# chengzhag/PanFusion

Hardware: NVIDIA B200
Metric: denoise-steps/sec (512x1024 pano + 8x512^2 views, 50-step DDIM) (higher is better)
Workload: dtype bf16

## Files before the change

panfusion_b200/csrc/fmha_tcgen05.cu:

```cuda
#include <stdlib.h>

#include "pf_common.cuh"

namespace pf {

constexpr int FA_BLOCK_M = 128;
constexpr int FA_BLOCK_N = 64;
constexpr int FA_THREADS = 192;
#ifndef PF_FA_POLY_EXP
#define PF_FA_POLY_EXP 0
#endif
#ifndef PF_FA_ALU_PACK
#define PF_FA_ALU_PACK 0
#endif
#ifndef PF_FA_POLY_DEFAULT
#define PF_FA_POLY_DEFAULT 0
#endif
constexpr bool FA_POLY_EXP = PF_FA_POLY_EXP != 0;
constexpr bool FA_ALU_PACK = PF_FA_ALU_PACK != 0;

struct FmhaParams {
  int B, H, Lq, Lk;
  float scale_log2;
  void* out;
  int out_ld;
  const float* bias;
  long long bias_bstride;
  int bias_ld;
  const uint8_t* bias_flags;
  long long flags_bstride;
  int flags_ld;
  const int* tile_off;
};

__device__ __forceinline__ float fast_exp2(float x) {
  float y;
  asm("ex2.approx.ftz.f32 %0, %1;" : "=f"(y) : "f"(x));
  return y;
}

__device__ __forceinline__ float poly_exp2(float x) {
  x = fmaxf(x, -125.0f);
  const float t = x + 12582912.0f;
  const float f = x - (t - 12582912.0f);
  float p = fmaf(f, 0.05517164f, 0.24261112f);
  p = fmaf(p, f, 0.69326099f);
  p = fmaf(p, f, 0.99992807f);
  return __int_as_float(__float_as_int(p) + (__float_as_int(t) << 23));
}

__device__ __forceinline__ void poly_exp2_pair(float x0, float x1, float& y0, float& y1) {
  const f32x2 x = pack_f2(fmaxf(x0, -125.0f), fmaxf(x1, -125.0f));
  const f32x2 magic = pack_f2(12582912.0f, 12582912.0f);
  const f32x2 t = add_f2(x, magic);
  const f32x2 r = add_f2(t, pack_f2(-12582912.0f, -12582912.0f));
  const f32x2 f = fma_f2(r, pack_f2(-1.0f, -1.0f), x);
  f32x2 p = fma_f2(f, pack_f2(0.05517164f, 0.05517164f), pack_f2(0.24261112f, 0.24261112f));
  p = fma_f2(p, f, pack_f2(0.69326099f, 0.69326099f));
  p = fma_f2(p, f, pack_f2(0.99992807f, 0.99992807f));
  float p0, p1, t0, t1;
  unpack_f2(p, p0, p1);
  unpack_f2(t, t0, t1);
  y0 = __int_as_float(__float_as_int(p0) + (__float_as_int(t0) << 23));
  y1 = __int_as_float(__float_as_int(p1) + (__float_as_int(t1) << 23));
}

__device__ __forceinline__ uint32_t pack_bf16_alu(float a, float b) {
  const uint32_t ua = __float_as_uint(a) + 0x8000u, ub = __float_as_uint(b) + 0x8000u;
  return __byte_perm(ua, ub, 0x7632);
}

template <bool BF16>
__device__ __forceinline__ uint32_t pack_prob(float a, float b) {
  if constexpr (BF16) return pack_bf16_alu(a, b);
  else return pack2<false>(a, b);
}

template <int D>
__host__ __device__ constexpr int fa_stages() { return D == 64 ? 2 : 4; }
template <int D>
__host__ __device__ constexpr int fmha_smem_bytes() {
  return FA_BLOCK_M * D * 2 + fa_stages<D>() * 2 * FA_BLOCK_N * D * 2 + FA_BLOCK_M * FA_BLOCK_N * 2 + 256;
}

template <int D, bool BF16, bool HAS_BIAS, int POLY_PAIRS>
__global__ void __launch_bounds__(FA_THREADS, 3)
fmha_fwd_kernel(const __grid_constant__ CUtensorMap tmQ, const __grid_constant__ CUtensorMap tmK,
                const __grid_constant__ CUtensorMap tmV, const FmhaParams p) {
  static_assert(D == 32 || D == 64, "head dim 32 (EPPA) or 64 (SD-2 UNet)");
  constexpr int STAGES = fa_stages<D>();
  constexpr int Q_BYTES = FA_BLOCK_M * D * 2;
  constexpr int KV_BYTES = FA_BLOCK_N * D * 2;
  constexpr int P_BYTES = FA_BLOCK_M * FA_BLOCK_N * 2;
  constexpr uint32_t SW_LAYOUT = (D == 64) ? 2u : 4u;
  constexpr uint32_t SW_ATOM_BYTES = (D == 64) ? 1024u : 512u;
  constexpr int TMEM_COLS = 128;
  constexpr uint32_t TM_S = 0, TM_O = 64;
  constexpr float RESCALE_THRESHOLD = 8.0f;

  extern __shared__ __align__(1024) uint8_t smem[];
  if ((smem_u32(smem) & 1023u) != 0) __trap();
  uint8_t* sQ = smem;
  uint8_t* sKV = sQ + Q_BYTES;
  uint8_t* sP = sKV + STAGES * 2 * KV_BYTES;
  uint64_t* bars = reinterpret_cast<uint64_t*>(sP + P_BYTES);
  uint64_t* q_full = bars;
  uint64_t* kv_full = bars + 1;
  uint64_t* kv_empty = kv_full + STAGES;
  uint64_t* s_full = kv_empty + STAGES;
  uint64_t* s_free = s_full + 1;
  uint64_t* p_full = s_free + 1;
  uint64_t* o_done = p_full + 1;
  uint32_t* tmem_ptr_smem = reinterpret_cast<uint32_t*>(o_done + 1);

  pdl_launch_dependents();
  const int warp = threadIdx.x >> 5, lane = threadIdx.x & 31;
  const int h = blockIdx.x % p.H;
  const int qt = blockIdx.x / p.H;
  const int b = blockIdx.y;
  const int q0 = qt * FA_BLOCK_M;
  const int n_tiles = (p.Lk + FA_BLOCK_N - 1) / FA_BLOCK_N;

  if (warp == 0 && lane == 0) {
    tma_prefetch_desc(&tmQ);
    tma_prefetch_desc(&tmK);
    tma_prefetch_desc(&tmV);
    mbar_init(q_full, 1);
    for (int s = 0; s < STAGES; ++s) {
      mbar_init(&kv_full[s], 1);
      mbar_init(&kv_empty[s], 1);
    }
    mbar_init(s_full, 1);
    mbar_init(s_free, 128);
    mbar_init(p_full, 128);
    mbar_init(o_done, 1);
    fence_barrier_init();
  }
  if (warp == 1) {
    tmem_alloc(tmem_ptr_smem, TMEM_COLS);
    tmem_relinquish();
  }
  tc_fence_before();
  __syncthreads();
  tc_fence_after();
  const uint32_t tmem_base = *tmem_ptr_smem;
  pdl_wait();

  if (warp == 0) {
    if (lane == 0) {
      mbar_expect_tx(q_full, Q_BYTES);
      tma_load_4d(sQ, &tmQ, q_full, 0, h, q0, b);
      for (int j = 0; j < n_tiles; ++j) {
        const int s = j % STAGES;
        mbar_wait(&kv_empty[s], ((j / STAGES) & 1) ^ 1);
        mbar_expect_tx(&kv_full[s], 2 * KV_BYTES);
        uint8_t* dst = sKV + s * 2 * KV_BYTES;
        tma_load_4d(dst, &tmK, &kv_full[s], 0, h, j * FA_BLOCK_N, b);
        tma_load_4d(dst + KV_BYTES, &tmV, &kv_full[s], 0, h, j * FA_BLOCK_N, b);
      }
    }
  } else if (warp == 1) {
    if (lane == 0) {
      constexpr uint32_t idesc_qk = make_idesc_f16(BF16 ? 1 : 0, FA_BLOCK_M, FA_BLOCK_N, 0, 0);
      constexpr uint32_t idesc_pv = make_idesc_f16(BF16 ? 1 : 0, FA_BLOCK_M, D, 0, 1);
      const uint64_t qdesc = make_smem_desc(smem_u32(sQ), 16, SW_ATOM_BYTES, SW_LAYOUT);
      const uint64_t pdesc = make_smem_desc(smem_u32(sP), 16, 1024, 2);
      auto issue_qk = [&](int j) {
        const int s = j % STAGES;
        mbar_wait(&kv_full[s], (j / STAGES) & 1);
        tc_fence_after();
        const uint64_t kdesc = make_smem_desc(smem_u32(sKV + s * 2 * KV_BYTES), 16, SW_ATOM_BYTES, SW_LAYOUT);
#pragma unroll
        for (int k = 0; k < D / 16; ++k) umma_f16(tmem_base + TM_S, qdesc + 2 * k, kdesc + 2 * k, idesc_qk, k != 0);
        umma_commit(s_full);
      };
      mbar_wait(q_full, 0);
      issue_qk(0);
      for (int j = 0; j < n_tiles; ++j) {
        mbar_wait(s_free, j & 1);
        tc_fence_after();
        if (j + 1 < n_tiles) issue_qk(j + 1);
        mbar_wait(p_full, j & 1);
        tc_fence_after();
        const int s = j % STAGES;
        const uint64_t vdesc =
            make_smem_desc(smem_u32(sKV + s * 2 * KV_BYTES + KV_BYTES), SW_ATOM_BYTES, SW_ATOM_BYTES, SW_LAYOUT);
#pragma unroll
        for (int k = 0; k < FA_BLOCK_N / 16; ++k) {
          umma_f16(tmem_base + TM_O, pdesc + 2 * k, vdesc + uint64_t((2 * SW_ATOM_BYTES * k) >> 4), idesc_pv,
                   (j | k) != 0 ? 1u : 0u);
        }
        umma_commit(o_done);
        umma_commit(&kv_empty[s]);
      }
    }
  } else {
    const int quarter = warp & 3;
    const int row = quarter * 32 + lane;
    const int q = q0 + row;
    const uint32_t lane_addr = tmem_base + (uint32_t(quarter * 32) << 16);
    constexpr float LOG2E = 1.4426950408889634f;
    float m_used = -INFINITY, l_run = 0.f;
    const float* bias_row = nullptr;
    const uint8_t* flag_row = nullptr;
    const int* off_row = nullptr;
    if constexpr (HAS_BIAS) {
      const int qq = q < p.Lq ? q : p.Lq - 1;
      if (p.tile_off) {
        off_row = p.tile_off + (long long)b * p.flags_bstride + (long long)qt * p.flags_ld;
        bias_row = p.bias + (quarter * (FA_BLOCK_N / 4) * 32 + lane) * 4;
      } else {
        bias_row = p.bias + (long long)b * p.bias_bstride + (long long)qq * p.bias_ld;
        if (p.bias_flags) flag_row = p.bias_flags + (long long)b * p.flags_bstride + (long long)qt * p.flags_ld;
      }
    }

    for (int j = 0; j < n_tiles; ++j) {
      const int k0 = j * FA_BLOCK_N;
      int toff = 0;
      if constexpr (HAS_BIAS) {
        if (off_row) toff = off_row[j];
      }
      mbar_wait(s_full, j & 1);
      tc_fence_after();
      float sv[FA_BLOCK_N];
      {
        uint32_t raw[32];
        tmem_ld32(lane_addr + TM_S, raw);
        tmem_ld_wait();
#pragma unroll
        for (int e = 0; e < 32; ++e) sv[e] = __uint_as_float(raw[e]);
        tmem_ld32(lane_addr + TM_S + 32, raw);
        tmem_ld_wait();
#pragma unroll
        for (int e = 0; e < 32; ++e) sv[32 + e] = __uint_as_float(raw[e]);
      }
      tc_fence_before();
      mbar_arrive(s_free);
      float sc = p.scale_log2, shift = 0.f;
      if constexpr (HAS_BIAS) {
        const bool constant_tile = off_row ? toff < 0 : (flag_row != nullptr && flag_row[j] != 0);
        if (constant_tile) {
          shift = -LOG2E;
        } else if (off_row || k0 + FA_BLOCK_N <= p.Lk) {
          const float4* b4 = off_row ? reinterpret_cast<const float4*>(bias_row + (long long)toff * (FA_BLOCK_M * FA_BLOCK_N))
                                     : reinterpret_cast<const float4*>(bias_row + k0);
          const int st4 = off_row ? 32 : 1;
#pragma unroll
          for (int e = 0; e < FA_BLOCK_N / 4; ++e) {
            const float4 t = __ldg(b4 + e * st4);
            sv[4 * e + 0] = fmaf(t.x, LOG2E, sv[4 * e + 0] * p.scale_log2);
            sv[4 * e + 1] = fmaf(t.y, LOG2E, sv[4 * e + 1] * p.scale_log2);
            sv[4 * e + 2] = fmaf(t.z, LOG2E, sv[4 * e + 2] * p.scale_log2);
            sv[4 * e + 3] = fmaf(t.w, LOG2E, sv[4 * e + 3] * p.scale_log2);
          }
          sc = 1.0f;
        } else {
#pragma unroll
          for (int e = 0; e < FA_BLOCK_N; ++e) {
            const float bv = (k0 + e < p.Lk) ? __ldg(bias_row + k0 + e) : 0.f;
            sv[e] = fmaf(bv, LOG2E, sv[e] * p.scale_log2);
          }
          sc = 1.0f;
        }
      }
      if (k0 + FA_BLOCK_N > p.Lk) {
#pragma unroll
        for (int e = 0; e < FA_BLOCK_N; ++e)
          if (k0 + e >= p.Lk) sv[e] = -INFINITY;
      }
      float mxs[8];
#pragma unroll
      for (int i = 0; i < 8; ++i) mxs[i] = sv[i];
#pragma unroll
      for (int e = 8; e < FA_BLOCK_N; ++e) mxs[e & 7] = fmaxf(mxs[e & 7], sv[e]);
      const float mx_raw = fmaxf(fmaxf(fmaxf(mxs[0], mxs[1]), fmaxf(mxs[2], mxs[3])),
                                 fmaxf(fmaxf(mxs[4], mxs[5]), fmaxf(mxs[6], mxs[7])));
      const float mx_tile = HAS_BIAS ? fmaf(mx_raw, sc, shift) : sc * mx_raw;
      const bool need = mx_tile > m_used + RESCALE_THRESHOLD;
      bool o_waited = false;
      if (__any_sync(0xffffffffu, need)) {
        const float m_new = need ? mx_tile : m_used;
        const float alpha = fast_exp2(m_used - m_new);
        if (j > 0) {
          mbar_wait(o_done, (j - 1) & 1);
          tc_fence_after();
          o_waited = true;
          uint32_t raw[16];
#pragma unroll 1
          for (int c = 0; c < D; c += 16) {
            tmem_ld16(lane_addr + TM_O + c, raw);
            tmem_ld_wait();
#pragma unroll
            for (int e = 0; e < 16; ++e) raw[e] = __float_as_uint(__uint_as_float(raw[e]) * alpha);
            tmem_st16(lane_addr + TM_O + c, raw);
          }
          tmem_st_wait();
        }
        l_run *= alpha;
        m_used = m_new;
      }
      f32x2 ps2[4];
#pragma unroll
      for (int i = 0; i < 4; ++i) ps2[i] = pack_f2(0.f, 0.f);
      const f32x2 sc2 = pack_f2(sc, sc), nm2 = HAS_BIAS ? pack_f2(shift - m_used, shift - m_used) : pack_f2(-m_used, -m_used);
      uint32_t pk[FA_BLOCK_N / 2];
#pragma unroll
      for (int e = 0; e < FA_BLOCK_N; e += 2) {
        float a0, a1;
        unpack_f2(fma_f2(pack_f2(sv[e], sv[e + 1]), sc2, nm2), a0, a1);
        float p0, p1;
        if (((e >> 1) & 7) < POLY_PAIRS) {
          poly_exp2_pair(a0, a1, p0, p1);
        } else {
          p0 = fast_exp2(a0);
          p1 = (FA_POLY_EXP && ((e >> 1) & 1)) ? poly_exp2(a1) : fast_exp2(a1);
        }
        ps2[(e >> 1) & 3] = add_f2(ps2[(e >> 1) & 3], pack_f2(p0, p1));
        pk[e >> 1] = FA_ALU_PACK ? pack_prob<BF16>(p0, p1) : pack2<BF16>(p0, p1);
      }
      {
        float lo, hi;
        unpack_f2(add_f2(add_f2(ps2[0], ps2[1]), add_f2(ps2[2], ps2[3])), lo, hi);
        l_run += lo + hi;
      }
      if (j > 0 && !o_waited) {
        mbar_wait(o_done, (j - 1) & 1);
        tc_fence_after();
      }
      {
        uint8_t* prow = sP + row * 128;
#pragma unroll
        for (int c = 0; c < 8; ++c) {
          uint4 v = make_uint4(pk[4 * c], pk[4 * c + 1], pk[4 * c + 2], pk[4 * c + 3]);
          *reinterpret_cast<uint4*>(prow + ((c ^ (row & 7)) << 4)) = v;
        }
      }
      fence_proxy_async_smem();
      tc_fence_before();
      mbar_arrive(p_full);
    }
    mbar_wait(o_done, (n_tiles - 1) & 1);
    tc_fence_after();
    {
      const float inv = 1.0f / l_run;
      uint16_t* orow = static_cast<uint16_t*>(p.out) + ((long long)b * p.Lq + q) * p.out_ld + h * D;
      uint32_t raw[32];
#pragma unroll
      for (int c = 0; c < D; c += 32) {
        tmem_ld32(lane_addr + TM_O + c, raw);
        tmem_ld_wait();
        if (q < p.Lq) {
#pragma unroll
          for (int e = 0; e < 32; e += 8) {
            uint4 v = make_uint4(pack2<BF16>(__uint_as_float(raw[e]) * inv, __uint_as_float(raw[e + 1]) * inv),
                                 pack2<BF16>(__uint_as_float(raw[e + 2]) * inv, __uint_as_float(raw[e + 3]) * inv),
                                 pack2<BF16>(__uint_as_float(raw[e + 4]) * inv, __uint_as_float(raw[e + 5]) * inv),
                                 pack2<BF16>(__uint_as_float(raw[e + 6]) * inv, __uint_as_float(raw[e + 7]) * inv));
            *reinterpret_cast<uint4*>(orow + c + e) = v;
          }
        }
      }
    }
    tc_fence_before();
  }
  __syncthreads();
  if (warp == 1) {
    tc_fence_after();
    tmem_dealloc(tmem_base, TMEM_COLS);
  }
}

static int make_qkv_tmap(CUtensorMap* tm, int dtype, const void* ptr, int B, int H, int L, int D, int ld,
                         long long bstride, int box_rows) {
  uint64_t dims[4] = {(uint64_t)D, (uint64_t)H, (uint64_t)L, (uint64_t)B};
  uint64_t str[3] = {(uint64_t)D * 2, (uint64_t)ld * 2, (uint64_t)bstride * 2};
  uint32_t box[4] = {(uint32_t)D, 1, (uint32_t)box_rows, 1};
  return make_tmap(tm, dtype, 4, ptr, dims, str, box, D == 64 ? 128 : 64);
}

template <int D, bool BF16, bool HAS_BIAS, int POLY_PAIRS>
static int launch_fmha(const pf_fmha_args* a, cudaStream_t st) {
  CUtensorMap tmQ, tmK, tmV;
  int rc;
  if ((rc = make_qkv_tmap(&tmQ, a->dtype, a->q, a->B, a->H, a->Lq, D, a->q_ld, a->q_bstride, FA_BLOCK_M))) return rc;
  if ((rc = make_qkv_tmap(&tmK, a->dtype, a->k, a->B, a->H, a->Lk, D, a->k_ld, a->k_bstride, FA_BLOCK_N))) return rc;
  if ((rc = make_qkv_tmap(&tmV, a->dtype, a->v, a->B, a->H, a->Lk, D, a->v_ld, a->v_bstride, FA_BLOCK_N))) return rc;
  FmhaParams p;
  p.B = a->B; p.H = a->H; p.Lq = a->Lq; p.Lk = a->Lk;
  p.scale_log2 = a->scale * 1.4426950408889634f;
  p.out = a->out; p.out_ld = a->out_ld;
  p.bias = a->bias; p.bias_bstride = a->bias_bstride; p.bias_ld = a->bias_ld;
  p.bias_flags = a->bias_flags; p.flags_bstride = a->flags_bstride; p.flags_ld = a->flags_ld;
  p.tile_off = a->bias_tile_off;
  auto kern = fmha_fwd_kernel<D, BF16, HAS_BIAS, POLY_PAIRS>;
  constexpr int SMEM = fmha_smem_bytes<D>();
  static bool attr_set = false;
  if (!attr_set) {
    rc = check_cuda(cudaFuncSetAttribute(kern, cudaFuncAttributeMaxDynamicSharedMemorySize, SMEM),
                    "cudaFuncSetAttribute(fmha)");
    if (rc) return rc;
    attr_set = true;
  }
  dim3 grid(((a->Lq + FA_BLOCK_M - 1) / FA_BLOCK_M) * a->H, a->B);
  if ((rc = check_cuda(launch_pdl(kern, grid, dim3(FA_THREADS), SMEM, st, tmQ, tmK, tmV, p), "launch(fmha)"))) return rc;
  PF_CHECK_LAUNCH("fmha_fwd_kernel");
  return PF_OK;
}

}

extern "C" int pf_fmha_fwd(const pf_fmha_args* a, void* stream) {
  using namespace pf;
  PF_CHECK_ARG(a != nullptr, "pf_fmha_fwd: null args");
  PF_CHECK_ARG(a->dtype == PF_BF16 || a->dtype == PF_F16, "pf_fmha_fwd: dtype must be PF_F16 or PF_BF16");
  PF_CHECK_ARG(a->q && a->k && a->v && a->out, "pf_fmha_fwd: null operand");
  PF_CHECK_ARG(a->head_dim == 32 || a->head_dim == 64, "pf_fmha_fwd: head_dim %d unsupported (32 or 64)", a->head_dim);
  PF_CHECK_ARG(a->B > 0 && a->B <= 65535 && a->H > 0 && a->Lq > 0 && a->Lk > 0, "pf_fmha_fwd: empty shape");
  PF_CHECK_ARG(a->q_ld % 8 == 0 && a->k_ld % 8 == 0 && a->v_ld % 8 == 0 && a->out_ld % 8 == 0,
               "pf_fmha_fwd: leading dims must be multiples of 8 elements");
  PF_CHECK_ARG(((uintptr_t)a->q & 15) == 0 && ((uintptr_t)a->k & 15) == 0 && ((uintptr_t)a->v & 15) == 0 &&
                   ((uintptr_t)a->out & 15) == 0,
               "pf_fmha_fwd: operands must be 16-byte aligned");
  PF_CHECK_ARG(!a->bias || a->bias_tile_off || (a->bias_ld % 4 == 0 && ((uintptr_t)a->bias & 15) == 0 && a->bias_ld >= a->Lk),
               "pf_fmha_fwd: bias must be 16-byte aligned with bias_ld %% 4 == 0");
  PF_CHECK_ARG(!a->bias_tile_off || (a->bias && ((uintptr_t)a->bias & 15) == 0 && !a->bias_flags && a->flags_ld > 0),
               "pf_fmha_fwd: a tile-packed bias needs the packed store in `bias`, flags_ld = tiles per row, no bias_flags");
  cudaStream_t st = static_cast<cudaStream_t>(stream);
  const bool bf = a->dtype == PF_BF16;
  const bool hb = a->bias != nullptr;
  static const int poly = [] {
    const char* e = getenv("PF_FA_POLY");
    return e ? atoi(e) : PF_FA_POLY_DEFAULT;
  }();
  if (a->head_dim == 64) {
    if (bf && !hb) {
      switch (poly) {
        case 2: return launch_fmha<64, true, false, 2>(a, st);
        case 3: return launch_fmha<64, true, false, 3>(a, st);
        case 4: return launch_fmha<64, true, false, 4>(a, st);
        default: return launch_fmha<64, true, false, 0>(a, st);
      }
    }
    if (bf) return launch_fmha<64, true, true, 0>(a, st);
    return hb ? launch_fmha<64, false, true, 0>(a, st) : launch_fmha<64, false, false, 0>(a, st);
  }
  if (bf) {
    if (hb) {
      switch (poly) {
        case 2: return launch_fmha<32, true, true, 2>(a, st);
        case 3: return launch_fmha<32, true, true, 3>(a, st);
        default: return launch_fmha<32, true, true, 0>(a, st);
      }
    }
    return launch_fmha<32, true, false, 0>(a, st);
  }
  return hb ? launch_fmha<32, false, true, 0>(a, st) : launch_fmha<32, false, false, 0>(a, st);
}
```

panfusion_b200/csrc/pf_common.cuh:

```cuda
#pragma once
#include <cuda.h>
#include <cuda_runtime.h>
#include <cuda_bf16.h>
#include <cuda_fp16.h>
#include <stdint.h>
#include <stdio.h>

#include "../../include/panfusion_b200.h"

namespace pf {

void set_error(const char* fmt, ...);
int  check_cuda(cudaError_t e, const char* what);
bool pdl_enabled();

#define PF_CHECK_ARG(cond, ...)                      \
  do {                                               \
    if (!(cond)) {                                   \
      ::pf::set_error(__VA_ARGS__);                  \
      return PF_ERR_INVALID;                         \
    }                                                \
  } while (0)

#define PF_CHECK_LAUNCH(what)                                         \
  do {                                                                \
    int _rc = ::pf::check_cuda(cudaGetLastError(), what);             \
    if (_rc) return _rc;                                              \
  } while (0)

int make_tmap(CUtensorMap* out, int dtype , int rank, const void* base,
              const uint64_t* dims, const uint64_t* strides_bytes, const uint32_t* box,
              int swizzle_bytes );

#ifdef __CUDACC__

__device__ __forceinline__ uint32_t smem_u32(const void* p) {
  return static_cast<uint32_t>(__cvta_generic_to_shared(p));
}

__device__ __forceinline__ void mbar_init(uint64_t* bar, uint32_t count) {
  asm volatile("mbarrier.init.shared::cta.b64 [%0], %1;" ::"r"(smem_u32(bar)), "r"(count) : "memory");
}
__device__ __forceinline__ void fence_barrier_init() {
  asm volatile("fence.mbarrier_init.release.cluster;" ::: "memory");
}
__device__ __forceinline__ void fence_proxy_async_smem() {
  asm volatile("fence.proxy.async.shared::cta;" ::: "memory");
}
__device__ __forceinline__ void mbar_expect_tx(uint64_t* bar, uint32_t bytes) {
  asm volatile("mbarrier.arrive.expect_tx.shared::cta.b64 _, [%0], %1;" ::"r"(smem_u32(bar)), "r"(bytes)
               : "memory");
}
__device__ __forceinline__ void mbar_arrive(uint64_t* bar) {
  asm volatile("mbarrier.arrive.shared::cta.b64 _, [%0];" ::"r"(smem_u32(bar)) : "memory");
}
__device__ __forceinline__ bool mbar_try_wait(uint64_t* bar, uint32_t parity) {
  uint32_t ok;
  asm volatile(
      "{\n\t.reg .pred p;\n\t"
      "mbarrier.try_wait.parity.shared::cta.b64 p, [%1], %2;\n\t"
      "selp.u32 %0, 1, 0, p;\n\t}"
      : "=r"(ok)
      : "r"(smem_u32(bar)), "r"(parity)
      : "memory");
  return ok != 0;
}
__device__ __forceinline__ void mbar_wait(uint64_t* bar, uint32_t parity) {
  if (mbar_try_wait(bar, parity)) return;
  const long long t0 = clock64();
  while (!mbar_try_wait(bar, parity)) {
    if (clock64() - t0 > 4000000000LL) {
      printf("pf: mbarrier wait timeout (block %d,%d thread %d)\n", blockIdx.x, blockIdx.y, threadIdx.x);
      __trap();
    }
  }
}

__device__ __forceinline__ void tma_prefetch_desc(const CUtensorMap* t) {
  asm volatile("prefetch.tensormap [%0];" ::"l"(t) : "memory");
}
__device__ __forceinline__ void tma_load_2d(void* dst, const CUtensorMap* t, uint64_t* bar, int c0, int c1) {
  asm volatile(
      "cp.async.bulk.tensor.2d.shared::cluster.global.mbarrier::complete_tx::bytes [%0], [%1, {%3, %4}], [%2];"
      ::"r"(smem_u32(dst)), "l"(t), "r"(smem_u32(bar)), "r"(c0), "r"(c1)
      : "memory");
}
__device__ __forceinline__ void tma_load_4d(void* dst, const CUtensorMap* t, uint64_t* bar, int c0, int c1,
                                            int c2, int c3) {
  asm volatile(
      "cp.async.bulk.tensor.4d.shared::cluster.global.mbarrier::complete_tx::bytes [%0], [%1, {%3, %4, %5, %6}], "
      "[%2];" ::"r"(smem_u32(dst)),
      "l"(t), "r"(smem_u32(bar)), "r"(c0), "r"(c1), "r"(c2), "r"(c3)
      : "memory");
}
__device__ __forceinline__ void tma_store_2d(const CUtensorMap* t, const void* src, int c0, int c1) {
  asm volatile("cp.async.bulk.tensor.2d.global.shared::cta.bulk_group [%0, {%2, %3}], [%1];" ::"l"(t),
               "r"(smem_u32(src)), "r"(c0), "r"(c1)
               : "memory");
}
__device__ __forceinline__ void tma_store_commit() { asm volatile("cp.async.bulk.commit_group;" ::: "memory"); }
__device__ __forceinline__ void tma_store_wait_read() { asm volatile("cp.async.bulk.wait_group.read 0;" ::: "memory"); }
__device__ __forceinline__ void named_bar_sync(int id, int nthreads) {
  asm volatile("bar.sync %0, %1;" ::"r"(id), "r"(nthreads) : "memory");
}

__device__ __forceinline__ void bulk_load_1d(void* dst, const void* src, uint32_t bytes, uint64_t* bar) {
  asm volatile(
      "cp.async.bulk.shared::cluster.global.mbarrier::complete_tx::bytes [%0], [%1], %2, [%3];" ::"r"(
          smem_u32(dst)),
      "l"(src), "r"(bytes), "r"(smem_u32(bar))
      : "memory");
}

__device__ __forceinline__ void tmem_alloc(uint32_t* smem_dst, uint32_t ncols) {
  asm volatile("tcgen05.alloc.cta_group::1.sync.aligned.shared::cta.b32 [%0], %1;" ::"r"(smem_u32(smem_dst)),
               "r"(ncols)
               : "memory");
}
__device__ __forceinline__ void tmem_relinquish() {
  asm volatile("tcgen05.relinquish_alloc_permit.cta_group::1.sync.aligned;" ::: "memory");
}
__device__ __forceinline__ void tmem_dealloc(uint32_t taddr, uint32_t ncols) {
  asm volatile("tcgen05.dealloc.cta_group::1.sync.aligned.b32 %0, %1;" ::"r"(taddr), "r"(ncols) : "memory");
}
__device__ __forceinline__ void tc_fence_before() {
  asm volatile("tcgen05.fence::before_thread_sync;" ::: "memory");
}
__device__ __forceinline__ void tc_fence_after() {
  asm volatile("tcgen05.fence::after_thread_sync;" ::: "memory");
}
__device__ __forceinline__ void umma_f16(uint32_t tmem_d, uint64_t adesc, uint64_t bdesc, uint32_t idesc,
                                         uint32_t accumulate) {
  asm volatile(
      "{\n\t.reg .pred p;\n\t"
      "setp.ne.b32 p, %4, 0;\n\t"
      "tcgen05.mma.cta_group::1.kind::f16 [%0], %1, %2, %3, p;\n\t}"
      ::"r"(tmem_d), "l"(adesc), "l"(bdesc), "r"(idesc), "r"(accumulate)
      : "memory");
}
__device__ __forceinline__ void umma_commit(uint64_t* bar) {
  asm volatile("tcgen05.commit.cta_group::1.mbarrier::arrive::one.shared::cluster.b64 [%0];" ::"r"(smem_u32(bar))
               : "memory");
}
__device__ __forceinline__ void tmem_ld_wait() { asm volatile("tcgen05.wait::ld.sync.aligned;" ::: "memory"); }

__device__ __forceinline__ void tmem_ld16(uint32_t taddr, uint32_t (&v)[16]) {
  asm volatile(
      "tcgen05.ld.sync.aligned.32x32b.x16.b32 {%0, %1, %2, %3, %4, %5, %6, %7, %8, %9, %10, %11, %12, %13, %14, "
      "%15}, [%16];"
      : "=r"(v[0]), "=r"(v[1]), "=r"(v[2]), "=r"(v[3]), "=r"(v[4]), "=r"(v[5]), "=r"(v[6]), "=r"(v[7]),
        "=r"(v[8]), "=r"(v[9]), "=r"(v[10]), "=r"(v[11]), "=r"(v[12]), "=r"(v[13]), "=r"(v[14]), "=r"(v[15])
      : "r"(taddr)
      : "memory");
}
__device__ __forceinline__ void tmem_ld32(uint32_t taddr, uint32_t (&v)[32]) {
  asm volatile(
      "tcgen05.ld.sync.aligned.32x32b.x32.b32 {%0, %1, %2, %3, %4, %5, %6, %7, %8, %9, %10, %11, %12, %13, %14, "
      "%15, %16, %17, %18, %19, %20, %21, %22, %23, %24, %25, %26, %27, %28, %29, %30, %31}, [%32];"
      : "=r"(v[0]), "=r"(v[1]), "=r"(v[2]), "=r"(v[3]), "=r"(v[4]), "=r"(v[5]), "=r"(v[6]), "=r"(v[7]),
        "=r"(v[8]), "=r"(v[9]), "=r"(v[10]), "=r"(v[11]), "=r"(v[12]), "=r"(v[13]), "=r"(v[14]), "=r"(v[15]),
        "=r"(v[16]), "=r"(v[17]), "=r"(v[18]), "=r"(v[19]), "=r"(v[20]), "=r"(v[21]), "=r"(v[22]), "=r"(v[23]),
        "=r"(v[24]), "=r"(v[25]), "=r"(v[26]), "=r"(v[27]), "=r"(v[28]), "=r"(v[29]), "=r"(v[30]), "=r"(v[31])
      : "r"(taddr)
      : "memory");
}

__device__ __forceinline__ void tmem_st32(uint32_t taddr, const uint32_t (&v)[32]) {
  asm volatile(
      "tcgen05.st.sync.aligned.32x32b.x32.b32 [%0], {%1, %2, %3, %4, %5, %6, %7, %8, %9, %10, %11, %12, %13, %14, %15, "
      "%16, %17, %18, %19, %20, %21, %22, %23, %24, %25, %26, %27, %28, %29, %30, %31, %32};"
      ::"r"(taddr), "r"(v[0]), "r"(v[1]), "r"(v[2]), "r"(v[3]), "r"(v[4]), "r"(v[5]), "r"(v[6]), "r"(v[7]), "r"(v[8]),
        "r"(v[9]), "r"(v[10]), "r"(v[11]), "r"(v[12]), "r"(v[13]), "r"(v[14]), "r"(v[15]), "r"(v[16]), "r"(v[17]),
        "r"(v[18]), "r"(v[19]), "r"(v[20]), "r"(v[21]), "r"(v[22]), "r"(v[23]), "r"(v[24]), "r"(v[25]), "r"(v[26]),
        "r"(v[27]), "r"(v[28]), "r"(v[29]), "r"(v[30]), "r"(v[31])
      : "memory");
}
__device__ __forceinline__ void tmem_st16(uint32_t taddr, const uint32_t (&v)[16]) {
  asm volatile(
      "tcgen05.st.sync.aligned.32x32b.x16.b32 [%0], {%1, %2, %3, %4, %5, %6, %7, %8, %9, %10, %11, %12, %13, %14, %15, "
      "%16};" ::"r"(taddr),
      "r"(v[0]), "r"(v[1]), "r"(v[2]), "r"(v[3]), "r"(v[4]), "r"(v[5]), "r"(v[6]), "r"(v[7]), "r"(v[8]), "r"(v[9]),
      "r"(v[10]), "r"(v[11]), "r"(v[12]), "r"(v[13]), "r"(v[14]), "r"(v[15])
      : "memory");
}
__device__ __forceinline__ void tmem_st_wait() { asm volatile("tcgen05.wait::st.sync.aligned;" ::: "memory"); }

__device__ __forceinline__ uint32_t cluster_ctarank() {
  uint32_t r;
  asm volatile("mov.u32 %0, %%cluster_ctarank;" : "=r"(r));
  return r;
}
__device__ __forceinline__ void cluster_sync_all() {
  asm volatile("barrier.cluster.arrive.release.aligned;\n\tbarrier.cluster.wait.acquire.aligned;" ::: "memory");
}
__device__ __forceinline__ void tma_load_2d_2sm(void* dst, const CUtensorMap* t, uint64_t* bar, int c0, int c1) {
  asm volatile(
      "cp.async.bulk.tensor.2d.cta_group::2.shared::cluster.global.mbarrier::complete_tx::bytes [%0], [%1, {%3, %4}], "
      "[%2];" ::"r"(smem_u32(dst)),
      "l"(t), "r"(smem_u32(bar) & 0xFEFFFFFFu), "r"(c0), "r"(c1)
      : "memory");
}
__device__ __forceinline__ void tmem_alloc_2sm(uint32_t* smem_dst, uint32_t ncols) {
  asm volatile("tcgen05.alloc.cta_group::2.sync.aligned.shared::cta.b32 [%0], %1;" ::"r"(smem_u32(smem_dst)),
               "r"(ncols)
               : "memory");
}
__device__ __forceinline__ void tmem_relinquish_2sm() {
  asm volatile("tcgen05.relinquish_alloc_permit.cta_group::2.sync.aligned;" ::: "memory");
}
__device__ __forceinline__ void tmem_dealloc_2sm(uint32_t taddr, uint32_t ncols) {
  asm volatile("tcgen05.dealloc.cta_group::2.sync.aligned.b32 %0, %1;" ::"r"(taddr), "r"(ncols) : "memory");
}
__device__ __forceinline__ void umma_f16_2sm(uint32_t tmem_d, uint64_t adesc, uint64_t bdesc, uint32_t idesc,
                                             uint32_t accumulate) {
  asm volatile(
      "{\n\t.reg .pred p;\n\t"
      "setp.ne.b32 p, %4, 0;\n\t"
      "tcgen05.mma.cta_group::2.kind::f16 [%0], %1, %2, %3, p;\n\t}"
      ::"r"(tmem_d), "l"(adesc), "l"(bdesc), "r"(idesc), "r"(accumulate)
      : "memory");
}
__device__ __forceinline__ void umma_commit_2sm(uint64_t* bar) {
  asm volatile(
      "tcgen05.commit.cta_group::2.mbarrier::arrive::one.shared::cluster.multicast::cluster.b64 [%0], %1;" ::"r"(
          smem_u32(bar)),
      "h"((uint16_t)3)
      : "memory");
}

__host__ __device__ constexpr uint32_t make_idesc_f16(int fmt, int M, int N, int a_mn_major, int b_mn_major) {
  return (1u << 4) | (uint32_t(fmt) << 7) | (uint32_t(fmt) << 10) | (uint32_t(a_mn_major) << 15) |
         (uint32_t(b_mn_major) << 16) | (uint32_t(N >> 3) << 17) | (uint32_t(M >> 4) << 24);
}

__device__ __forceinline__ uint64_t make_smem_desc(uint32_t saddr, uint32_t lbo_bytes, uint32_t sbo_bytes,
                                                   uint32_t layout_type) {
  return uint64_t((saddr & 0x3FFFFu) >> 4) | (uint64_t(lbo_bytes >> 4) << 16) | (uint64_t(sbo_bytes >> 4) << 32) |
         (uint64_t(1) << 46) | (uint64_t(layout_type) << 61);
}

template <typename T>
struct Cvt;
template <>
struct Cvt<float> {
  static __device__ __forceinline__ float to_f(float v) { return v; }
  static __device__ __forceinline__ float from_f(float v) { return v; }
};
template <>
struct Cvt<__nv_bfloat16> {
  static __device__ __forceinline__ float to_f(__nv_bfloat16 v) { return __bfloat162float(v); }
  static __device__ __forceinline__ __nv_bfloat16 from_f(float v) { return __float2bfloat16_rn(v); }
};
template <>
struct Cvt<__half> {
  static __device__ __forceinline__ float to_f(__half v) { return __half2float(v); }
  static __device__ __forceinline__ __half from_f(float v) { return __float2half_rn(v); }
};

template <bool BF16>
__device__ __forceinline__ uint32_t pack2(float a, float b) {
  if constexpr (BF16) {
    __nv_bfloat162 t = __floats2bfloat162_rn(a, b);
    return *reinterpret_cast<uint32_t*>(&t);
  } else {
    __half2 t = __floats2half2_rn(a, b);
    return *reinterpret_cast<uint32_t*>(&t);
  }
}
template <bool BF16>
__device__ __forceinline__ float2 unpack2(uint32_t w) {
  if constexpr (BF16) {
    __nv_bfloat162 t = *reinterpret_cast<__nv_bfloat162*>(&w);
    return __bfloat1622float2(t);
  } else {
    __half2 t = *reinterpret_cast<__half2*>(&w);
    return __half22float2(t);
  }
}

__device__ __forceinline__ void pdl_launch_dependents() { asm volatile("griddepcontrol.launch_dependents;" ::: "memory"); }
__device__ __forceinline__ void pdl_wait() { asm volatile("griddepcontrol.wait;" ::: "memory"); }

__device__ __forceinline__ float ex2_approx(float x) {
  float y;
  asm("ex2.approx.ftz.f32 %0, %1;" : "=f"(y) : "f"(x));
  return y;
}
__device__ __forceinline__ float rcp_approx(float x) {
  float y;
  asm("rcp.approx.ftz.f32 %0, %1;" : "=f"(y) : "f"(x));
  return y;
}
__device__ __forceinline__ float silu_f(float x) {
  return x * rcp_approx(1.0f + ex2_approx(-1.4426950408889634f * x));
}
__device__ __forceinline__ float erf_as_f(float x) {
  const float ax = fabsf(x);
  const float t = rcp_approx(fmaf(0.3275911f, ax, 1.0f));
  float p = fmaf(1.061405429f, t, -1.453152027f);
  p = fmaf(p, t, 1.421413741f);
  p = fmaf(p, t, -0.284496736f);
  p = fmaf(p, t, 0.254829592f);
  const float r = fmaf(-p * t, ex2_approx(ax * (ax * -1.4426950408889634f)), 1.0f);
  return copysignf(r, x);
}
__device__ __forceinline__ float gelu_erf_f(float x) {
  const float hx = 0.5f * x;
  return fmaf(hx, erf_as_f(x * 0.70710678118654752440f), hx);
}

typedef unsigned long long f32x2;
__device__ __forceinline__ f32x2 pack_f2(float a, float b) {
  f32x2 r;
  asm("mov.b64 %0, {%1, %2};" : "=l"(r) : "f"(a), "f"(b));
  return r;
}
__device__ __forceinline__ void unpack_f2(f32x2 v, float& a, float& b) {
  asm("mov.b64 {%0, %1}, %2;" : "=f"(a), "=f"(b) : "l"(v));
}
__device__ __forceinline__ f32x2 fma_f2(f32x2 a, f32x2 b, f32x2 c) {
  f32x2 d;
  asm("fma.rn.f32x2 %0, %1, %2, %3;" : "=l"(d) : "l"(a), "l"(b), "l"(c));
  return d;
}
__device__ __forceinline__ f32x2 mul_f2(f32x2 a, f32x2 b) {
  f32x2 d;
  asm("mul.rn.f32x2 %0, %1, %2;" : "=l"(d) : "l"(a), "l"(b));
  return d;
}
__device__ __forceinline__ f32x2 add_f2(f32x2 a, f32x2 b) {
  f32x2 d;
  asm("add.rn.f32x2 %0, %1, %2;" : "=l"(d) : "l"(a), "l"(b));
  return d;
}
__device__ __forceinline__ void geglu_pair(float a0, float a1, float g0, float g1, float ba0, float ba1, float bg0, float bg1,
                                           float& o0, float& o1) {
  const f32x2 x = add_f2(pack_f2(g0, g1), pack_f2(bg0, bg1));
  const f32x2 val = add_f2(pack_f2(a0, a1), pack_f2(ba0, ba1));
  const f32x2 xs = mul_f2(x, pack_f2(0.70710678118654752440f, 0.70710678118654752440f));
  float xs0, xs1;
  unpack_f2(xs, xs0, xs1);
  const float ax0 = fabsf(xs0), ax1 = fabsf(xs1);
  const f32x2 ax = pack_f2(ax0, ax1);
  float d0, d1;
  unpack_f2(fma_f2(pack_f2(0.3275911f, 0.3275911f), ax, pack_f2(1.0f, 1.0f)), d0, d1);
  const f32x2 t = pack_f2(rcp_approx(d0), rcp_approx(d1));
  f32x2 p = fma_f2(pack_f2(1.061405429f, 1.061405429f), t, pack_f2(-1.453152027f, -1.453152027f));
  p = fma_f2(p, t, pack_f2(1.421413741f, 1.421413741f));
  p = fma_f2(p, t, pack_f2(-0.284496736f, -0.284496736f));
  p = fma_f2(p, t, pack_f2(0.254829592f, 0.254829592f));
  float e0, e1;
  unpack_f2(mul_f2(ax, mul_f2(ax, pack_f2(-1.4426950408889634f, -1.4426950408889634f))), e0, e1);
  const f32x2 ex = pack_f2(ex2_approx(e0), ex2_approx(e1));
  const f32x2 npt = mul_f2(mul_f2(p, pack_f2(-1.0f, -1.0f)), t);
  float r0, r1;
  unpack_f2(fma_f2(npt, ex, pack_f2(1.0f, 1.0f)), r0, r1);
  const f32x2 erfv = pack_f2(copysignf(r0, xs0), copysignf(r1, xs1));
  const f32x2 hx = mul_f2(x, pack_f2(0.5f, 0.5f));
  unpack_f2(mul_f2(val, fma_f2(hx, erfv, hx)), o0, o1);
}

__device__ __forceinline__ float warp_sum(float v) {
#pragma unroll
  for (int o = 16; o > 0; o >>= 1) v += __shfl_xor_sync(0xffffffffu, v, o);
  return v;
}
__device__ __forceinline__ float warp_max(float v) {
#pragma unroll
  for (int o = 16; o > 0; o >>= 1) v = fmaxf(v, __shfl_xor_sync(0xffffffffu, v, o));
  return v;
}

#endif

template <typename... KArgs, typename... Args>
inline cudaError_t launch_pdl(void (*kern)(KArgs...), dim3 grid, dim3 block, size_t smem, cudaStream_t st, Args&&... args) {
  cudaLaunchConfig_t cfg = {};
  cfg.gridDim = grid;
  cfg.blockDim = block;
  cfg.dynamicSmemBytes = smem;
  cfg.stream = st;
  cudaLaunchAttribute attr[1];
  attr[0].id = cudaLaunchAttributeProgrammaticStreamSerialization;
  attr[0].val.programmaticStreamSerializationAllowed = 1;
  cfg.attrs = attr;
  cfg.numAttrs = pdl_enabled() ? 1 : 0;
  return cudaLaunchKernelEx(&cfg, kern, static_cast<KArgs>(args)...);
}

}
```

Baseline: 37.32.

## Add warp-specialized FA4-style d64 attention kernel for long unbiased key sequences

Adds a new head-dim-64 attention kernel used when there is no bias and at least 4096 keys. It uses 128-wide key tiles, two query tiles per CTA with ping-pong QK/PV issue, P kept in tensor memory as the A operand of the PV MMA, and register reallocation between producer and softmax warps. It also skips rescaling the output until the running max grows past a threshold. The aim is to overlap tensor-core work with the exp/softmax work and cut shared-memory traffic for P. In exchange it adds a larger TMEM allocation and the lazy rescale changes numerics slightly.

```diff
diff --git a/panfusion_b200/csrc/fmha_d64.cu b/panfusion_b200/csrc/fmha_d64.cu
--- /dev/null
+++ b/panfusion_b200/csrc/fmha_d64.cu
@@ -0,0 +1,289 @@
+#include "pf_common.cuh"
+
+namespace pf {
+
+namespace {
+
+constexpr int F2_D = 64;
+constexpr int F2_BLOCK_M = 128;
+constexpr int F2_BLOCK_N = 128;
+constexpr int F2_Q_TILES = 2;
+constexpr int F2_THREADS = 128 * (1 + F2_Q_TILES);
+constexpr int F2_STAGES = F2_Q_TILES == 2 ? 3 : 2;
+constexpr int F2_Q_BYTES = F2_BLOCK_M * F2_D * 2;
+constexpr int F2_KV_BYTES = F2_BLOCK_N * F2_D * 2;
+constexpr int F2_SMEM = F2_Q_TILES * F2_Q_BYTES + F2_STAGES * 2 * F2_KV_BYTES + 256 + 1024;
+constexpr uint32_t F2_TMEM_COLS = 256 * F2_Q_TILES;
+constexpr uint32_t F2_TM_S = 0, F2_TM_P = 128, F2_TM_O = 192, F2_TM_TILE = 256;
+constexpr float F2_RESCALE_THRESHOLD = 8.0f;
+constexpr int F2_POLY_PAIRS = 0;
+
+template <bool BF16>
+__global__ void __launch_bounds__(F2_THREADS, 2 / F2_Q_TILES)
+fmha_d64_kernel(const __grid_constant__ CUtensorMap tmQ, const __grid_constant__ CUtensorMap tmK,
+                const __grid_constant__ CUtensorMap tmV, int H, int Lq, int Lk, float scale_log2, void* out, int out_ld) {
+  extern __shared__ uint8_t smem_raw[];
+  uint8_t* smem = reinterpret_cast<uint8_t*>((reinterpret_cast<uintptr_t>(smem_raw) + 1023) & ~uintptr_t(1023));
+  uint8_t* sQ = smem;
+  uint8_t* sKV = sQ + F2_Q_TILES * F2_Q_BYTES;
+  uint64_t* bars = reinterpret_cast<uint64_t*>(sKV + F2_STAGES * 2 * F2_KV_BYTES);
+  uint64_t* q_full = bars;
+  uint64_t* kv_full = q_full + 1;
+  uint64_t* kv_empty = kv_full + F2_STAGES;
+  uint64_t* s_full = kv_empty + F2_STAGES;
+  uint64_t* s_free = s_full + 2;
+  uint64_t* p_full = s_free + 2;
+  uint64_t* o_done = p_full + 2;
+  uint32_t* tmem_ptr_smem = reinterpret_cast<uint32_t*>(o_done + 2);
+
+  pdl_launch_dependents();
+  const int warp = threadIdx.x >> 5, lane = threadIdx.x & 31;
+  const int h = blockIdx.x % H;
+  const int q0 = (blockIdx.x / H) * (F2_Q_TILES * F2_BLOCK_M);
+  const int b = blockIdx.y;
+  const int n_qt = (F2_Q_TILES == 2 && q0 + F2_BLOCK_M < Lq) ? 2 : 1;
+  const int n_tiles = (Lk + F2_BLOCK_N - 1) / F2_BLOCK_N;
+
+  if (warp == 0 && lane == 0) {
+    tma_prefetch_desc(&tmQ);
+    tma_prefetch_desc(&tmK);
+    tma_prefetch_desc(&tmV);
+    mbar_init(q_full, 1);
+    for (int s = 0; s < F2_STAGES; ++s) {
+      mbar_init(&kv_full[s], 1);
+      mbar_init(&kv_empty[s], 1);
+    }
+    for (int t = 0; t < 2; ++t) {
+      mbar_init(&s_full[t], 1);
+      mbar_init(&s_free[t], 128);
+      mbar_init(&p_full[t], 128);
+      mbar_init(&o_done[t], 1);
+    }
+    fence_barrier_init();
+  }
+  if (warp == 1) {
+    tmem_alloc(tmem_ptr_smem, F2_TMEM_COLS);
+    tmem_relinquish();
+  }
+  tc_fence_before();
+  __syncthreads();
+  tc_fence_after();
+  const uint32_t tmem_base = *tmem_ptr_smem;
+  pdl_wait();
+
+  if (warp < 4) {
+    setmaxnreg_dec<56>();
+    if (warp == 0 && lane == 0) {
+      mbar_expect_tx(q_full, n_qt * F2_Q_BYTES);
+      for (int t = 0; t < n_qt; ++t) tma_load_4d(sQ + t * F2_Q_BYTES, &tmQ, q_full, 0, h, q0 + t * F2_BLOCK_M, b);
+      for (int j = 0; j < n_tiles; ++j) {
+        const int s = j % F2_STAGES;
+        mbar_wait(&kv_empty[s], ((j / F2_STAGES) & 1) ^ 1);
+        mbar_expect_tx(&kv_full[s], 2 * F2_KV_BYTES);
+        uint8_t* dst = sKV + s * 2 * F2_KV_BYTES;
+        tma_load_4d(dst, &tmK, &kv_full[s], 0, h, j * F2_BLOCK_N, b);
+        tma_load_4d(dst + F2_KV_BYTES, &tmV, &kv_full[s], 0, h, j * F2_BLOCK_N, b);
+      }
+    } else if (warp == 1 && lane == 0) {
+      constexpr uint32_t idesc_qk = make_idesc_f16(BF16 ? 1 : 0, F2_BLOCK_M, F2_BLOCK_N, 0, 0);
+      constexpr uint32_t idesc_pv = make_idesc_f16(BF16 ? 1 : 0, F2_BLOCK_M, F2_D, 0, 1);
+      auto issue_qk = [&](int j, int t) {
+        const uint64_t qdesc = make_smem_desc(smem_u32(sQ + t * F2_Q_BYTES), 16, 1024, 2);
+        const uint64_t kdesc = make_smem_desc(smem_u32(sKV + (j % F2_STAGES) * 2 * F2_KV_BYTES), 16, 1024, 2);
+#pragma unroll
+        for (int k = 0; k < F2_D / 16; ++k)
+          umma_f16(tmem_base + t * F2_TM_TILE + F2_TM_S, qdesc + 2 * k, kdesc + 2 * k, idesc_qk, k != 0);
+        umma_commit(&s_full[t]);
+      };
+      auto issue_pv = [&](int j, int t) {
+        const uint64_t vdesc = make_smem_desc(smem_u32(sKV + (j % F2_STAGES) * 2 * F2_KV_BYTES + F2_KV_BYTES), 1024, 1024, 2);
+        const uint32_t tp = tmem_base + t * F2_TM_TILE + F2_TM_P;
+#pragma unroll
+        for (int k = 0; k < F2_BLOCK_N / 16; ++k)
+          umma_f16_tmem_a(tmem_base + t * F2_TM_TILE + F2_TM_O, tp + 8 * k, vdesc + uint64_t((2 * 1024 * k) >> 4), idesc_pv,
+                          (j | k) != 0 ? 1u : 0u);
+        umma_commit(&o_done[t]);
+      };
+      mbar_wait(q_full, 0);
+      mbar_wait(&kv_full[0], 0);
+      tc_fence_after();
+      for (int t = 0; t < n_qt; ++t) issue_qk(0, t);
+      for (int j = 0; j < n_tiles; ++j) {
+        const bool next = j + 1 < n_tiles;
+        if (next) {
+          mbar_wait(&kv_full[(j + 1) % F2_STAGES], ((j + 1) / F2_STAGES) & 1);
+          tc_fence_after();
+        }
+        for (int t = 0; t < n_qt && next; ++t) {
+          mbar_wait(&s_free[t], j & 1);
+          tc_fence_after();
+          issue_qk(j + 1, t);
+        }
+        for (int t = 0; t < n_qt; ++t) {
+          mbar_wait(&p_full[t], j & 1);
+          tc_fence_after();
+          issue_pv(j, t);
+        }
+        umma_commit(&kv_empty[j % F2_STAGES]);
+      }
+    }
+  } else {
+    setmaxnreg_inc<F2_Q_TILES == 2 ? 224 : 200>();
+    const int t = (warp >> 2) - 1;
+    if (t < n_qt) {
+      const int quarter = warp & 3;
+      const int row = quarter * 32 + lane;
+      const int q = q0 + t * F2_BLOCK_M + row;
+      const uint32_t lane_addr = tmem_base + (uint32_t(quarter * 32) << 16) + t * F2_TM_TILE;
+      float m_used = -INFINITY, l_run = 0.f;
+      for (int j = 0; j < n_tiles; ++j) {
+        const int k0 = j * F2_BLOCK_N;
+        mbar_wait(&s_full[t], j & 1);
+        tc_fence_after();
+        float sv[F2_BLOCK_N];
+        {
+          uint32_t raw[4][32];
+#pragma unroll
+          for (int c = 0; c < 4; ++c) tmem_ld32(lane_addr + F2_TM_S + 32 * c, raw[c]);
+          tmem_ld_wait();
+#pragma unroll
+          for (int c = 0; c < 4; ++c)
+#pragma unroll
+            for (int e = 0; e < 32; ++e) sv[32 * c + e] = __uint_as_float(raw[c][e]);
+        }
+        tc_fence_before();
+        mbar_arrive(&s_free[t]);
+        if (k0 + F2_BLOCK_N > Lk) {
+#pragma unroll
+          for (int e = 0; e < F2_BLOCK_N; ++e)
+            if (k0 + e >= Lk) sv[e] = -INFINITY;
+        }
+        float mxs[8];
+#pragma unroll
+        for (int i = 0; i < 8; ++i) mxs[i] = sv[i];
+#pragma unroll
+        for (int e = 8; e < F2_BLOCK_N; ++e) mxs[e & 7] = fmaxf(mxs[e & 7], sv[e]);
+        const float mx_tile = scale_log2 * fmaxf(fmaxf(fmaxf(mxs[0], mxs[1]), fmaxf(mxs[2], mxs[3])),
+                                                 fmaxf(fmaxf(mxs[4], mxs[5]), fmaxf(mxs[6], mxs[7])));
+        const bool need = mx_tile > m_used + F2_RESCALE_THRESHOLD;
+        bool o_waited = false;
+        if (__any_sync(0xffffffffu, need)) {
+          const float m_new = need ? mx_tile : m_used;
+          const float alpha = ex2_approx(m_used - m_new);
+          if (j > 0) {
+            mbar_wait(&o_done[t], (j - 1) & 1);
+            tc_fence_after();
+            o_waited = true;
+            uint32_t raw[16];
+#pragma unroll 1
+            for (int c = 0; c < F2_D; c += 16) {
+              tmem_ld16(lane_addr + F2_TM_O + c, raw);
+              tmem_ld_wait();
+#pragma unroll
+              for (int e = 0; e < 16; ++e) raw[e] = __float_as_uint(__uint_as_float(raw[e]) * alpha);
+              tmem_st16(lane_addr + F2_TM_O + c, raw);
+            }
+            tmem_st_wait();
+          }
+          l_run *= alpha;
+          m_used = m_new;
+        }
+        f32x2 ps2[4];
+#pragma unroll
+        for (int i = 0; i < 4; ++i) ps2[i] = pack_f2(0.f, 0.f);
+        const f32x2 sc2 = pack_f2(scale_log2, scale_log2), nm2 = pack_f2(-m_used, -m_used);
+        uint32_t pk[F2_BLOCK_N / 2];
+#pragma unroll
+        for (int e = 0; e < F2_BLOCK_N; e += 2) {
+          float a0, a1, p0, p1;
+          unpack_f2(fma_f2(pack_f2(sv[e], sv[e + 1]), sc2, nm2), a0, a1);
+          if (((e >> 1) & 7) < F2_POLY_PAIRS) {
+            poly_exp2_pair(a0, a1, p0, p1);
+          } else {
+            p0 = ex2_approx(a0);
+            p1 = ex2_approx(a1);
+          }
+          ps2[(e >> 1) & 3] = add_f2(ps2[(e >> 1) & 3], pack_f2(p0, p1));
+          pk[e >> 1] = pack2<BF16>(p0, p1);
+        }
+        {
+          float lo, hi;
+          unpack_f2(add_f2(add_f2(ps2[0], ps2[1]), add_f2(ps2[2], ps2[3])), lo, hi);
+          l_run += lo + hi;
+        }
+        if (j > 0 && !o_waited) {
+          mbar_wait(&o_done[t], (j - 1) & 1);
+          tc_fence_after();
+        }
+        {
+          const uint32_t(&pk0)[32] = *reinterpret_cast<const uint32_t(*)[32]>(&pk[0]);
+          const uint32_t(&pk1)[32] = *reinterpret_cast<const uint32_t(*)[32]>(&pk[32]);
+          tmem_st32(lane_addr + F2_TM_P, pk0);
+          tmem_st32(lane_addr + F2_TM_P + 32, pk1);
+        }
+        tmem_st_wait();
+        tc_fence_before();
+        mbar_arrive(&p_full[t]);
+      }
+      mbar_wait(&o_done[t], (n_tiles - 1) & 1);
+      tc_fence_after();
+      const float inv = 1.0f / l_run;
+      uint16_t* orow = static_cast<uint16_t*>(out) + ((long long)b * Lq + q) * out_ld + h * F2_D;
+      uint32_t raw[2][32];
+      tmem_ld32(lane_addr + F2_TM_O, raw[0]);
+      tmem_ld32(lane_addr + F2_TM_O + 32, raw[1]);
+      tmem_ld_wait();
+      if (q < Lq) {
+#pragma unroll
+        for (int c = 0; c < 2; ++c)
+#pragma unroll
+          for (int e = 0; e < 32; e += 8) {
+            const uint32_t* r = raw[c] + e;
+            uint4 v = make_uint4(pack2<BF16>(__uint_as_float(r[0]) * inv, __uint_as_float(r[1]) * inv),
+                                 pack2<BF16>(__uint_as_float(r[2]) * inv, __uint_as_float(r[3]) * inv),
+                                 pack2<BF16>(__uint_as_float(r[4]) * inv, __uint_as_float(r[5]) * inv),
+                                 pack2<BF16>(__uint_as_float(r[6]) * inv, __uint_as_float(r[7]) * inv));
+            *reinterpret_cast<uint4*>(orow + 32 * c + e) = v;
+          }
+      }
+      tc_fence_before();
+    }
+  }
+  __syncthreads();
+  if (warp == 1) {
+    tc_fence_after();
+    tmem_dealloc(tmem_base, F2_TMEM_COLS);
+  }
+}
+
+template <bool BF16>
+int launch(const pf_fmha_args* a, cudaStream_t st) {
+  CUtensorMap tmQ, tmK, tmV;
+  int rc;
+  if ((rc = make_qkv_tmap(&tmQ, a->dtype, a->q, a->B, a->H, a->Lq, F2_D, a->q_ld, a->q_bstride, F2_BLOCK_M))) return rc;
+  if ((rc = make_qkv_tmap(&tmK, a->dtype, a->k, a->B, a->H, a->Lk, F2_D, a->k_ld, a->k_bstride, F2_BLOCK_N))) return rc;
+  if ((rc = make_qkv_tmap(&tmV, a->dtype, a->v, a->B, a->H, a->Lk, F2_D, a->v_ld, a->v_bstride, F2_BLOCK_N))) return rc;
+  auto kern = fmha_d64_kernel<BF16>;
+  static bool attr_set = false;
+  if (!attr_set) {
+    if ((rc = check_cuda(cudaFuncSetAttribute(kern, cudaFuncAttributeMaxDynamicSharedMemorySize, F2_SMEM),
+                         "cudaFuncSetAttribute(fmha_d64)")))
+      return rc;
+    attr_set = true;
+  }
+  dim3 grid(((a->Lq + F2_Q_TILES * F2_BLOCK_M - 1) / (F2_Q_TILES * F2_BLOCK_M)) * a->H, a->B);
+  if ((rc = check_cuda(launch_pdl(kern, grid, dim3(F2_THREADS), F2_SMEM, st, tmQ, tmK, tmV, a->H, a->Lq, a->Lk,
+                                  a->scale * 1.4426950408889634f, a->out, a->out_ld),
+                       "launch(fmha_d64)")))
+    return rc;
+  PF_CHECK_LAUNCH("fmha_d64_kernel");
+  return PF_OK;
+}
+
+}
+
+int launch_fmha_d64(const pf_fmha_args* a, cudaStream_t st) {
+  return a->dtype == PF_BF16 ? launch<true>(a, st) : launch<false>(a, st);
+}
+
+}
diff --git a/panfusion_b200/csrc/fmha_tcgen05.cu b/panfusion_b200/csrc/fmha_tcgen05.cu
--- a/panfusion_b200/csrc/fmha_tcgen05.cu
+++ b/panfusion_b200/csrc/fmha_tcgen05.cu
@@ -47,22 +47,6 @@
   p = fmaf(p, f, 0.69326099f);
   p = fmaf(p, f, 0.99992807f);
   return __int_as_float(__float_as_int(p) + (__float_as_int(t) << 23));
-}
-
-__device__ __forceinline__ void poly_exp2_pair(float x0, float x1, float& y0, float& y1) {
-  const f32x2 x = pack_f2(fmaxf(x0, -125.0f), fmaxf(x1, -125.0f));
-  const f32x2 magic = pack_f2(12582912.0f, 12582912.0f);
-  const f32x2 t = add_f2(x, magic);
-  const f32x2 r = add_f2(t, pack_f2(-12582912.0f, -12582912.0f));
-  const f32x2 f = fma_f2(r, pack_f2(-1.0f, -1.0f), x);
-  f32x2 p = fma_f2(f, pack_f2(0.05517164f, 0.05517164f), pack_f2(0.24261112f, 0.24261112f));
-  p = fma_f2(p, f, pack_f2(0.69326099f, 0.69326099f));
-  p = fma_f2(p, f, pack_f2(0.99992807f, 0.99992807f));
-  float p0, p1, t0, t1;
-  unpack_f2(p, p0, p1);
-  unpack_f2(t, t0, t1);
-  y0 = __int_as_float(__float_as_int(p0) + (__float_as_int(t0) << 23));
-  y1 = __int_as_float(__float_as_int(p1) + (__float_as_int(t1) << 23));
 }
 
 __device__ __forceinline__ uint32_t pack_bf16_alu(float a, float b) {
@@ -371,7 +355,7 @@
   }
 }
 
-static int make_qkv_tmap(CUtensorMap* tm, int dtype, const void* ptr, int B, int H, int L, int D, int ld,
+int make_qkv_tmap(CUtensorMap* tm, int dtype, const void* ptr, int B, int H, int L, int D, int ld,
                          long long bstride, int box_rows) {
   uint64_t dims[4] = {(uint64_t)D, (uint64_t)H, (uint64_t)L, (uint64_t)B};
   uint64_t str[3] = {(uint64_t)D * 2, (uint64_t)ld * 2, (uint64_t)bstride * 2};
@@ -407,6 +391,9 @@
   PF_CHECK_LAUNCH("fmha_fwd_kernel");
   return PF_OK;
 }
+
+int launch_fmha_d64(const pf_fmha_args* a, cudaStream_t st);
+constexpr int FA_D64_MIN_KEYS = 4096;
 
 }
 
@@ -434,15 +421,8 @@
     return e ? atoi(e) : PF_FA_POLY_DEFAULT;
   }();
   if (a->head_dim == 64) {
-    if (bf && !hb) {
-      switch (poly) {
-        case 2: return launch_fmha<64, true, false, 2>(a, st);
-        case 3: return launch_fmha<64, true, false, 3>(a, st);
-        case 4: return launch_fmha<64, true, false, 4>(a, st);
-        default: return launch_fmha<64, true, false, 0>(a, st);
-      }
-    }
-    if (bf) return launch_fmha<64, true, true, 0>(a, st);
+    if (!hb && a->Lk >= FA_D64_MIN_KEYS) return launch_fmha_d64(a, st);
+    if (bf) return hb ? launch_fmha<64, true, true, 0>(a, st) : launch_fmha<64, true, false, 0>(a, st);
     return hb ? launch_fmha<64, false, true, 0>(a, st) : launch_fmha<64, false, false, 0>(a, st);
   }
   if (bf) {
diff --git a/panfusion_b200/csrc/pf_common.cuh b/panfusion_b200/csrc/pf_common.cuh
--- a/panfusion_b200/csrc/pf_common.cuh
+++ b/panfusion_b200/csrc/pf_common.cuh
@@ -31,6 +31,8 @@
 int make_tmap(CUtensorMap* out, int dtype , int rank, const void* base,
               const uint64_t* dims, const uint64_t* strides_bytes, const uint32_t* box,
               int swizzle_bytes );
+int make_qkv_tmap(CUtensorMap* tm, int dtype, const void* ptr, int B, int H, int L, int D, int ld, long long bstride,
+                  int box_rows);
 
 #ifdef __CUDACC__
 
@@ -136,6 +138,15 @@
       "setp.ne.b32 p, %4, 0;\n\t"
       "tcgen05.mma.cta_group::1.kind::f16 [%0], %1, %2, %3, p;\n\t}"
       ::"r"(tmem_d), "l"(adesc), "l"(bdesc), "r"(idesc), "r"(accumulate)
+      : "memory");
+}
+__device__ __forceinline__ void umma_f16_tmem_a(uint32_t tmem_d, uint32_t tmem_a, uint64_t bdesc, uint32_t idesc,
+                                                uint32_t accumulate) {
+  asm volatile(
+      "{\n\t.reg .pred p;\n\t"
+      "setp.ne.b32 p, %4, 0;\n\t"
+      "tcgen05.mma.cta_group::1.kind::f16 [%0], [%1], %2, %3, p;\n\t}"
+      ::"r"(tmem_d), "r"(tmem_a), "l"(bdesc), "r"(idesc), "r"(accumulate)
       : "memory");
 }
 __device__ __forceinline__ void umma_commit(uint64_t* bar) {
@@ -280,6 +291,11 @@
 
 __device__ __forceinline__ void pdl_launch_dependents() { asm volatile("griddepcontrol.launch_dependents;" ::: "memory"); }
 __device__ __forceinline__ void pdl_wait() { asm volatile("griddepcontrol.wait;" ::: "memory"); }
+
+template <int N>
+__device__ __forceinline__ void setmaxnreg_dec() { asm volatile("setmaxnreg.dec.sync.aligned.u32 %0;" ::"n"(N)); }
+template <int N>
+__device__ __forceinline__ void setmaxnreg_inc() { asm volatile("setmaxnreg.inc.sync.aligned.u32 %0;" ::"n"(N)); }
 
 __device__ __forceinline__ float ex2_approx(float x) {
   float y;
@@ -360,6 +376,22 @@
   unpack_f2(mul_f2(val, fma_f2(hx, erfv, hx)), o0, o1);
 }
 
+__device__ __forceinline__ void poly_exp2_pair(float x0, float x1, float& y0, float& y1) {
+  const f32x2 x = pack_f2(fmaxf(x0, -125.0f), fmaxf(x1, -125.0f));
+  const f32x2 magic = pack_f2(12582912.0f, 12582912.0f);
+  const f32x2 t = add_f2(x, magic);
+  const f32x2 r = add_f2(t, pack_f2(-12582912.0f, -12582912.0f));
+  const f32x2 f = fma_f2(r, pack_f2(-1.0f, -1.0f), x);
+  f32x2 p = fma_f2(f, pack_f2(0.05517164f, 0.05517164f), pack_f2(0.24261112f, 0.24261112f));
+  p = fma_f2(p, f, pack_f2(0.69326099f, 0.69326099f));
+  p = fma_f2(p, f, pack_f2(0.99992807f, 0.99992807f));
+  float p0, p1, t0, t1;
+  unpack_f2(p, p0, p1);
+  unpack_f2(t, t0, t1);
+  y0 = __int_as_float(__float_as_int(p0) + (__float_as_int(t0) << 23));
+  y1 = __int_as_float(__float_as_int(p1) + (__float_as_int(t1) << 23));
+}
+
 __device__ __forceinline__ float warp_sum(float v) {
 #pragma unroll
   for (int o = 16; o > 0; o >>= 1) v += __shfl_xor_sync(0xffffffffu, v, o);
```

New measurement: 37.38 (median of 6 runs). About the same (+0.2%).
